# dropbox/lepton

Hardware: AMD Instinct MI355X
Metric: encode+decode MB/s (JPEG bytes/sec), bit-exact round trip (higher is better)
Workload: dtype int16/u8 (integer coder, no floating point)

## Files before the change

### lepton_amd/csrc/lep_enc5.h

```cpp
#pragma once
#include "lep_v3.h"
#ifdef LEP5_DEBUG
#include <cstdio>
#endif

namespace lep5 {
using namespace lep3;

constexpr int kRows = 64, kClasses = 10;
constexpr int kPRows = 63 + 14;
constexpr int kStreams = 2 * kRows * kClasses;
WDEV int stream_id(int ci, int row, int k) { return (ci * kRows + row) * kClasses + k; }
constexpr int kCoefSlice = 12 * 11 + 10 + 1;
constexpr int kSignSlice = 48, kNzSlice = 6 * 32, kEdgeNzSlice = 8 * 12, kDcSlice = 17 * 11 + 10 + 1;
constexpr uint32_t kThreshWords = 2u * 256 * 8 * 128;

WDEV uint32_t coef_entry(uint32_t vlow, int nres, int len, int bsr, int k, int u) {
    return vlow | ((uint32_t)nres << 10) | ((uint32_t)len << 14) | ((uint32_t)bsr << 18) | ((uint32_t)k << 23) | ((uint32_t)u << 27);
}
WDEV int coef_units(int len, int nres) { return ((len < 11 ? len + 1 : 11) + nres + 3) >> 2; }
WDEV uint32_t thresh_entry(uint32_t tbits, int n, int pcls, int lt, int u) {
    return tbits | ((uint32_t)n << 10) | ((uint32_t)pcls << 14) | ((uint32_t)lt << 23) | ((uint32_t)u << 27);
}
constexpr int kKeyRec = 4, kNzRec = 8, kEnRec = 8, kDcRec = 24;
// ... 413 lines not shown
                    if (overflow) status[sd.slot] = 100;
                } else { ws->low = bc.low; ws->stage = bc.stage; ws->q24 = bc.q24; ws->count = bc.count; ws->nst = bc.nst; ws->pos = bc.pos; }
            }
        }
    }
}


constexpr uint32_t kWarm5 = 16384;
struct WChunk5 { uint32_t q_guess, q_end, shifts, q_start, t_start, keep, keep_bits, carry, pos_end, pad[7]; };
static_assert(sizeof(WChunk5) == 64, "one record per (segment, chunk)");
WDEV uint32_t chunk_first_bin(uint32_t nbins, int k, int K) { return (uint32_t)(((uint64_t)nbins * (uint32_t)k) / (uint32_t)K); }
WDEV int range_step(uint32_t& q24, uint32_t bit, uint32_t prob) {
#if LEP_ON_GPU
    const uint32_t s = __umulhi(q24, prob);
#else
    const uint32_t s = (uint32_t)(((uint64_t)q24 * prob) >> 32);
#endif
    const uint32_t q = q24 >> 24;
    const uint32_t n = bit ? q - s : s + 1;
    const int f = __builtin_clz(n);
    q24 = (n << f) - (1u << 24);
    return f - 24;
}
template <class F, class G>
WDEV void for_bins(const uint16_t* list, uint32_t b0, uint32_t b1, F&& f, G&& g) {
    uint32_t i = b0;
    for (; i < b1 && (i & 31u); ++i) { const uint32_t e = list[i]; f((e >> 8) & 1u, e & 255u); g(); }
    if (i + 32 <= b1) {
        const uint32_t* b = reinterpret_cast<const uint32_t*>(list);
        U4 n0 = ld4(b + (i >> 1)), n1 = ld4(b + (i >> 1) + 4), n2 = ld4(b + (i >> 1) + 8), n3 = ld4(b + (i >> 1) + 12);
#define LEP5_BINS8(v)                                                                                      \
    f((v.x >> 8) & 1u, v.x & 255u); f((v.x >> 24) & 1u, (v.x >> 16) & 255u);                               \
    f((v.y >> 8) & 1u, v.y & 255u); f((v.y >> 24) & 1u, (v.y >> 16) & 255u); g();                          \
    f((v.z >> 8) & 1u, v.z & 255u); f((v.z >> 24) & 1u, (v.z >> 16) & 255u);                               \
    f((v.w >> 8) & 1u, v.w & 255u); f((v.w >> 24) & 1u, (v.w >> 16) & 255u); g();
        for (; i + 32 <= b1; i += 32) {
            const U4 g0 = n0, g1 = n1, g2 = n2, g3 = n3;
            const uint32_t* nx = b + (i >> 1) + 16;
            n0 = ld4(nx); n1 = ld4(nx + 4); n2 = ld4(nx + 8); n3 = ld4(nx + 12);
            LEP5_BINS8(g0) LEP5_BINS8(g1) LEP5_BINS8(g2) LEP5_BINS8(g3)
        }
#undef LEP5_BINS8
    }
    for (; i < b1; ++i) { const uint32_t e = list[i]; f((e >> 8) & 1u, e & 255u); g(); }
}
WDEV void range_run(const uint16_t* list, uint32_t b0, uint32_t b1, bool first, bool last, uint32_t& q24, uint32_t& shifts) {
    uint32_t t = 0, q = q24;
    if (first) t += (uint32_t)range_step(q, 0, 128);
    for_bins(list, b0, b1, [&](uint32_t bit, uint32_t prob) { t += (uint32_t)range_step(q, bit, prob); }, []() {});
    if (last) for (int i = 0; i < 32; ++i) t += (uint32_t)range_step(q, 0, 128);
    shifts = t; q24 = q;
}
WDEV void wchunk_range_lane(const SegPlan5& P, const uint16_t* bins, WChunk5* rec, int k, int K, uint32_t warm = kWarm5) {
    if (P.status) return;
    const uint16_t* list = bins + P.bins_off;
    const uint32_t b0 = chunk_first_bin(P.nbins, k, K), b1 = chunk_first_bin(P.nbins, k + 1, K);
    uint32_t q24 = 254u << 24, sh = 0;
    if (k > 0) {
        const bool from_start = b0 <= warm;
        range_run(list, from_start ? 0u : b0 - warm, b0, from_start, false, q24, sh);
    }
    rec->q_guess = q24;
    range_run(list, b0, b1, k == 0, k + 1 == K, q24, sh);
    rec->q_end = q24; rec->shifts = sh;
}
WDEV uint32_t bytes_at(uint32_t T) { return T >= 24 ? ((T - 24) >> 3) + 1 : 0u; }
WDEV int count_at(uint32_t T) { return (int)T - 24 - 8 * (int)bytes_at(T); }
WDEV void wchunk_link_lane(const SegPlan5& P, const uint16_t* bins, WChunk5* recs, int K) {
    if (P.status) return;
    const uint16_t* list = bins + P.bins_off;
    uint32_t T = 0, q = 254u << 24;
    for (int k = 0; k < K; ++k) {
        WChunk5& r = recs[k];
        if (k > 0 && r.q_guess != q) {
            uint32_t q24 = q, sh = 0;
            range_run(list, chunk_first_bin(P.nbins, k, K), chunk_first_bin(P.nbins, k + 1, K), false, k + 1 == K, q24, sh);
            r.q_end = q24; r.shifts = sh;
        }
        r.q_start = q; r.t_start = T;
        q = r.q_end; T += r.shifts;
    }
}
WDEV void wchunk_code_lane(const SegPlan5& P, const uint16_t* bins, const SegDev& sd, uint8_t* streams, WChunk5* rec, int k, int K) {
    if (P.status) return;
    const uint16_t* list = bins + P.bins_off;
    const uint32_t b0 = chunk_first_bin(P.nbins, k, K), b1 = chunk_first_bin(P.nbins, k + 1, K);
    BoolEnc5 bc;
    bc.init(streams + sd.stream_off, sd.stream_cap);
    bc.q24 = rec->q_start;
    bc.pos = bytes_at(rec->t_start); bc.count = count_at(rec->t_start); bc.floor_ = bc.pos;
    if (k == 0) { bc.bin(0, 128); bc.flush(); }
    for_bins(list, b0, b1, [&](uint32_t bit, uint32_t prob) { bc.bin(bit, prob); }, [&]() { bc.flush(); });
    bc.flush();
    if (k + 1 == K) for (int i = 0; i < 32; ++i) { bc.bin(0, 128); if ((i & 3) == 3) bc.flush(); }
    bc.flush();
    for (; bc.nst; --bc.nst) { if (bc.pos < bc.cap) bc.out[bc.pos] = (uint8_t)(bc.stage >> (8 * (bc.nst - 1))); ++bc.pos; }
    rec->keep = (uint32_t)bc.low; rec->keep_bits = (uint32_t)(32 + bc.count); rec->carry = bc.carry_out; rec->pos_end = bc.pos;
}
WDEV void add_back(uint8_t* out, uint32_t cap, uint32_t x, uint32_t v) {
    while (v && x > 0) {
        --x;
        if (x < cap) { const uint32_t t = out[x] + v; out[x] = (uint8_t)t; v = t >> 8; }
        else v = 0;
    }
}
WDEV void wchunk_stitch_lane(const SegPlan5& P, const SegDev& sd, uint8_t* streams, uint32_t* stream_len, int32_t* status, const WChunk5* recs, int K) {
    if (P.status) { status[sd.slot] = P.status; return; }
    uint8_t* out = streams + sd.stream_off;
    const uint32_t cap = sd.stream_cap;
    for (int k = 0; k + 1 < K; ++k) {
        const WChunk5& r = recs[k];
        const uint32_t X = r.keep_bits ? r.keep << (32 - r.keep_bits) : 0u;
        uint32_t carry = 0;
        for (int j = 3; j >= 0; --j) {
            const uint32_t x = r.pos_end + (uint32_t)j, add = (X >> (24 - 8 * j)) & 255u;
            if (x < cap) { const uint32_t t = out[x] + add + carry; out[x] = (uint8_t)t; carry = t >> 8; }
            else carry = 0;
        }
        add_back(out, cap, r.pos_end, carry);
        add_back(out, cap, recs[k + 1].t_start >= 24 ? bytes_at(recs[k + 1].t_start) : 0u, recs[k + 1].carry);
    }
    uint32_t pos = recs[K - 1].pos_end;
    const bool overflow = pos >= cap;
    if (!overflow && pos && (out[pos - 1] & 0xe0u) == 0xc0u) { out[pos] = 0; ++pos; }
    stream_len[sd.slot] = pos;
    if (overflow) status[sd.slot] = 100;
}

enum { kCount = 0, kEmit = 1, kGather = 2 };

#ifndef LEP_ENC5_GATHER_ROW_FLUSH
#define LEP_ENC5_GATHER_ROW_FLUSH 1
#endif
#if LEP_ENC5_GATHER_ROW_FLUSH
struct BinAcc {
    uint32_t lw;
    uint32_t fu;
    uint32_t blo, bhi;
};
#else
typedef uint32_t BinAcc;
#endif

struct Walk5Shared {
    uint32_t cur[32 * 65];
    uint16_t TB[8 * 65];
    uint16_t q[64];
    uint8_t thr[64];
    uint16_t errx[2 * 64];
    uint32_t tcur[2 * 8];
// ... 939 lines not shown
```

### lepton_amd/csrc/lep_gpu.hip

```cpp
#include <hip/hip_runtime.h>

#include <algorithm>
#include <cstdio>
#include <cstdlib>
#include <cstring>
#include <mutex>
#include <string>
#include <vector>

#include "../../include/lepton_mi355x.h"
#include "lep_buffers.h"

#define LEP_DEV __device__ __forceinline__
#include "lep_core.h"
#include "lep_enc3.h"
#include "lep_dec4.h"
#include "lep_enc5.h"
#include "lep_huff.h"
#include "lep_huffdec.h"
#include "lep_huffdec_simt.h"
#include "lep_huff_simt.h"
#include "lep_huffprog.h"
#include "lep_huffprog_simt.h"
#include "lep_huffprogdec.h"
// ... 131 lines not shown
    __shared__ lep4::Dec4Shared sh;
    const int s = blockIdx.x, lane = threadIdx.x;
    const SegDev seg = segs[s];
    lep4::Dec4Resume* rec = recs + seg.slot;
    const int state = rec->state;
    if (state != lep4::kRowsFresh && state != lep4::kRowsRunning) return;
    const ImageDev* img = images + seg.image;
    uint32_t* model = models + (size_t)s * kModelStride;
    NSum* ns = ns_area + ns_offsets[s];
    if (state == lep4::kRowsFresh) {
        reset_segment_state<lep3::kModelWords>(model, ns, img->ns_total, lane);
        __syncthreads();
    }
    lep4::Dec4WaveT<SCMASK> w;
#ifdef LEP_PROF
    w.prof_begin(&g_prof4[s & 8191][0]);
#endif
    w.run_rows(img, seg, model, ns, &sh, streams + seg.stream_off, stream_len[seg.slot], rec, lds_save + (size_t)seg.slot * kRowsLdsWords, band_mcu_rows);
}


template <int MODE, int NW>
__global__ __launch_bounds__(64 * NW) void lep_enc5_walk_kernel(const ImageDev* __restrict__ images, const SegDev* __restrict__ segs, NSum* ns_all,
                                                         const uint64_t* __restrict__ ns_off, lep5::SegPlan5* plans, uint8_t* arena, uint16_t* bins,
                                                         uint32_t* counts, int part, int nparts) {
    lep5::Walk5Shared* sh = reinterpret_cast<lep5::Walk5Shared*>(lep5::lep5_lds);
    const int s = blockIdx.x;
    const SegDev seg = segs[s];
    lep5::SegPlan5* P = plans + s;
    if (MODE == lep5::kGather && P->status) return;
    lep5::Walk5<MODE, NW> w;
    const int rc = w.run(images + seg.image, seg, ns_all + ns_off[s], sh, P, arena, bins, (int)(threadIdx.x >> 6), part, nparts);
    if (threadIdx.x >= 64) return;
    if (MODE == lep5::kCount) lep5::export_counts(w, sh, counts + (size_t)s * lep5::kCountWords);
    if (threadIdx.x == 0) {
        if (MODE == lep5::kEmit) P->status = rc;
        if (MODE == lep5::kGather && part + 1 == nparts) P->nbins = w.nbins;
    }
}
template <int PHASE>
__global__ __launch_bounds__(64) void lep_enc5_wchunk_kernel(const lep5::SegPlan5* __restrict__ plans, const uint16_t* __restrict__ bins, const SegDev* __restrict__ segs,
                                                         int nseg, int K, lep5::WChunk5* recs, uint8_t* streams, uint32_t* stream_len, int32_t* status, uint32_t* nbins_out) {
    const int id = (int)(blockIdx.x * 64 + threadIdx.x);
    if (PHASE == 0 || PHASE == 2) {
        const int seg = id / K, k = id - seg * K;
        if (seg >= nseg) return;
        if (PHASE == 2) __builtin_amdgcn_s_setprio(3);
        if (PHASE == 0) lep5::wchunk_range_lane(plans[seg], bins, recs + (size_t)seg * K + k, k, K);
        else lep5::wchunk_code_lane(plans[seg], bins, segs[seg], streams, recs + (size_t)seg * K + k, k, K);
    } else {
        if (id >= nseg) return;
        if (PHASE == 1) { status[segs[id].slot] = 0; nbins_out[segs[id].slot] = plans[id].nbins; lep5::wchunk_link_lane(plans[id], bins, recs + (size_t)id * K, K); }
        else lep5::wchunk_stitch_lane(plans[id], segs[id], streams, stream_len, status, recs + (size_t)id * K, K);
    }
}
__global__ void lep_enc5_plan_kernel(const uint32_t* __restrict__ counts, lep5::SegPlan5* plans, int nseg) {
    const int s = (int)(blockIdx.x * blockDim.x + threadIdx.x);
    if (s < nseg) lep5::plan_segment(counts + (size_t)s * lep5::kCountWords, plans + s);
}
__global__ __launch_bounds__(64) void lep_enc5_offsets_kernel(lep5::SegPlan5* plans, int nseg, uint64_t* totals) {
    uint64_t a = 0, b = 0;
    for (int s0 = 0; s0 < nseg; s0 += 64) {
        const int s = s0 + (int)threadIdx.x;
        const uint32_t ab = s < nseg ? plans[s].arena_bytes : 0u, bc = s < nseg ? plans[s].bins_cap : 0u;
        int oa, ob;
        const int va = (int)(ab >> 8), vb = (int)(bc >> 7);
        const int ta = lepwave::wave_excl_scan(&va, &oa), tb = lepwave::wave_excl_scan(&vb, &ob);
        if (s < nseg) { plans[s].arena_off = a + ((uint64_t)(uint32_t)oa << 8); plans[s].bins_off = b + ((uint64_t)(uint32_t)ob << 7); }
        a += (uint64_t)(uint32_t)ta << 8; b += (uint64_t)(uint32_t)tb << 7;
    }
    if (threadIdx.x == 0) { totals[0] = a; totals[1] = b; }
}
__global__ void lep_enc5_fill_kernel(uint4* p, size_t n16, uint32_t v) {
    const uint4 x = make_uint4(v, v, v, v);
    for (size_t i = blockIdx.x * (size_t)blockDim.x + threadIdx.x; i < n16; i += (size_t)gridDim.x * blockDim.x) p[i] = x;
}
__global__ __launch_bounds__(64) void lep_enc5_bucket_kernel(const lep5::SegPlan5* __restrict__ plans, uint8_t* arena) {
    __shared__ lep5::BucketShared sh;
    lep5::bucket_wave(plans + blockIdx.x, arena, &sh);
}
struct Fold5CoefShared { uint16_t slice[lep5::kCoefSlice * 64]; };
__global__ __launch_bounds__(64) void lep_enc5_fold_coef_kernel(const lep5::SegPlan5* __restrict__ plans, uint8_t* arena, int nseg, int groups) {
    __shared__ Fold5CoefShared shc;
    const int grp = (int)blockIdx.x % groups, job = (int)blockIdx.x / groups;
    const int ci = job / 630, row = (job % 630) / 10, k = job % 10;
    const int sid = lep5::stream_id(ci, row, k), seg = grp * 64 + (int)threadIdx.x;
    const bool work = seg < nseg && !plans[seg].status && plans[seg].cnt[sid] != 0;
    if (!__ballot(work)) return;
    lep5::fold_coef_wave(plans, arena, grp * 64, nseg, sid, reinterpret_cast<lep5::FoldShared*>(&shc));
}
struct Fold5SmallShared { uint16_t slice[lep5::kEdgeNzSlice * 64]; };
__global__ __launch_bounds__(64) void lep_enc5_fold_small_kernel(const lep5::SegPlan5* __restrict__ plans, uint8_t* arena, uint32_t* thresh_models, int nseg, int groups, int job0) {
    __shared__ Fold5SmallShared shs;
    lep5::FoldShared* sh = reinterpret_cast<lep5::FoldShared*>(&shs);
    const int grp = (int)blockIdx.x % groups;
    int job = (int)blockIdx.x / groups + job0;
    const int seg0 = grp * 64;
    if (job < 2) { lep5::fold_sign_wave(plans, arena, seg0, nseg, job, sh); return; }
    job -= 2;
    if (job < 12) { const int ci = job / 6, lt = 2 + job % 6; lep5::fold_thresh_wave(plans, arena, thresh_models, seg0, nseg, lep5::stream_id(ci, 63, lt), ci, sh); return; }
    job -= 12;
    lep5::fold_edgenz_wave(plans, arena, seg0, nseg, job / 16, (job / 8) & 1, job & 7, sh);
}
constexpr int kFold5SmallJobs = 2 + 12 + 32;
__global__ __launch_bounds__(64) void lep_enc5_fold_big_kernel(const lep5::SegPlan5* __restrict__ plans, uint8_t* arena, int nseg, int groups, int job0) {
    __shared__ lep5::FoldShared sh;
// ... 191 lines not shown
    __shared__ lephuff::SimtShared sh;
    extern __shared__ __attribute__((aligned(16))) unsigned char simt_columns[];
    const lephuff::SimtWave w = waves[blockIdx.x];
    lephuff::simt_guess_or_settle(images + w.image, &sh, si + w.image, in + si[w.image].first, out + si[w.image].first, w.first_sub, settle, slots,
                                  reinterpret_cast<lephuff::SimtColumns*>(simt_columns));
}
__global__ __launch_bounds__(64) void lep_huffman_simt_place_kernel(const lephuff::HuffDecImage* __restrict__ images, lephuff::SimtImage* si, const lephuff::SimtSub* sub,
                                                                    lephuff::SimtPlace* place, int passes, lephuff::HuffDecRow* rows, const lephuff::SimtSlots* slots) {
    const int i = (int)blockIdx.x;
    lephuff::simt_place(images + i, si + i, sub + si[i].first, place + si[i].first, passes, rows, slots);
}
__global__ __launch_bounds__(64) void lep_huffman_simt_write_kernel(const lephuff::HuffDecImage* __restrict__ images, lephuff::SimtImage* si, const lephuff::SimtWave* waves,
                                                                    const lephuff::SimtSub* sub, const lephuff::SimtPlace* place, lephuff::HuffDecRow* rows) {
    __shared__ lephuff::SimtShared sh;
    __shared__ lephuff::SimtTile tile;
    const lephuff::SimtWave w = waves[blockIdx.x];
    lephuff::simt_write(images + w.image, &sh, &tile, si + w.image, sub + si[w.image].first, place + si[w.image].first, rows, w.first_sub);
}
__global__ void lep_huffman_simt_finish_kernel(const lephuff::HuffDecImage* __restrict__ images, int nimg, lephuff::HuffDecRow* rows, const lephuff::SimtImage* si) {
    const int i = (int)(blockIdx.x * blockDim.x + threadIdx.x);
    if (i < nimg) lephuff::simt_finish(images + i, si + i, rows);
}

}

struct lep_gpu {
    int device = 0;
    hipStream_t stream = nullptr;
    hipEvent_t ev0 = nullptr, ev1 = nullptr;
    bool timed = false;
    bool released = false;
    int enc5_min = 8;
    hipStream_t stream2 = nullptr, stream3 = nullptr;
    hipEvent_t ev_fork = nullptr, ev_join = nullptr, ev_join3 = nullptr;
    int huffprog_pipeline = 1;
    int huffprog_split = 0;
    int huffprogdec_rst = 1;
    uint32_t huffprogdec_rst_floor = lephuff::kRstPieceFloor;
    int huffprogdec_win = 1;
    int huffprog_simt = 1;
    int huffprog_simt_rst = 1;
    uint32_t huffprog_forms[4] = {0, 0, 0, 0};
    int cut_progressive = 0;
    int stream_pack = 1;
    int huffenc_simt = 1;
    int simt_sub_bits = 0;
    int huffprog_pipeline_max = 16384;
    int enc5_waves = 2;
    int enc5_parts = 8;
    hipEvent_t ev_part[8] = {nullptr, nullptr, nullptr, nullptr, nullptr, nullptr, nullptr, nullptr};
    long enc5_wlanes = 131072;
    int enc5_wmaxseg = 4096;
    int enc5_wchunks = 64;
    int enc5_gather_wgs = 0;
    int enc5_fold_apart = 0;
    size_t enc5_scratch_max = ~(size_t)0;
    hipEvent_t ev_stage[8] = {nullptr, nullptr, nullptr, nullptr, nullptr, nullptr, nullptr, nullptr};
    int nstage = 0;
    int enc_waves = 0;
    int enc_pair_max = 1280;
    int dec_company = 0;
    int dec_waves = 0;
    std::string err;
    const char* last_kernel = "";
    char simt_name[112] = "";
    struct Vmm {
        bool on = false;
        size_t chunk = (size_t)512 << 20;
        hipMemAllocationProp prop;
        hipMemAccessDesc access;
        std::vector<hipMemGenericAllocationHandle_t> pool;
        size_t mapped_total = 0, creates = 0, releases = 0;
    } vmm;
    enum Ws {
        W_ENC5_ENTRIES,
        W_ENC5_BINLIST,
        W_MODELS, W_MODELS_1,
        W_NS, W_NS_1,
        W_TRIMMED,
        W_META = W_TRIMMED, W_META_1,
        W_ROWS, W_ROWS_1,
        W_ENC5_PLANS,
        W_ENC5_WCHUNKS,
        W_BLOCKS, W_STREAMS, W_LENS,
        W_HUFF, W_HUFF_1,
        W_HUFFENC, W_HUFFENC_1,
        W_HUFFPROG, W_HUFFPROG_1,
        W_HUFFPROGSIMT, W_HUFFPROGSIMT_1,
        W_HUFFSEQ, W_HUFFSEQ_1,
        W_HUFFPROGDEC,
        W_HUFFPROGRST,
        W_HUFFDEC,
        W_HUFFPAR,
        W_PACK, W_PACK_1,
        W_COUNT
    };
    lepbuf::DevBuf<> ws[W_COUNT];
    int cur = 0;
    struct RowsSession {
        bool open = false;
        int nseg = 0, waves = 4;
        hipStream_t st = nullptr;
        const ImageDev* d_img = nullptr; const SegDev* d_seg = nullptr; const uint64_t* d_nsoff = nullptr;
        uint32_t* d_models = nullptr; NSum* d_ns = nullptr;
        const uint8_t* d_streams = nullptr; const uint32_t* d_stream_len = nullptr;
        std::vector<lep4::Dec4Resume> h_recs;
// ... 106 lines not shown
        if (hipMemMap(b.va + b.mapped, V.chunk, 0, h, 0) != hipSuccess) { (void)hipGetLastError(); (void)hipMemRelease(h); g->err = "hipMemMap failed"; return LEP_GPU_ERROR; }
        b.chunks.push_back(h); b.mapped += V.chunk; V.mapped_total += V.chunk;
    }
    if (b.mapped > old) HIPCHK(g, hipMemSetAccess(b.va + old, b.mapped - old, &V.access, 1));
    w.set(b.va, b.mapped);
    return 0;
}
static int ensure(lep_gpu* g, Workspace& w, size_t need, bool may_release = true) {
    if (w.cap >= need) return 0;
    if (g->vmm.on && (need >= ((size_t)32 << 20) || w.v.va)) {
        if (!w.v.va) HIPCHK(g, w.release());
        return vmm_ensure(g, w, need, may_release);
    }
    hipError_t e = w.ensure(need, need / 8);
    if (e != hipSuccess && may_release) {
        (void)hipGetLastError();
        release_idle_caches(g);
        e = w.ensure(need);
    }
    if (e != hipSuccess) { g->err = std::string("hipMalloc: ") + hipGetErrorString(e); return LEP_GPU_ERROR; }
    return 0;
}

#include "lep_derive.h"


constexpr int kEnc5NoMemory = -1000;
static int launch_enc5(lep_gpu* g, const ImageDev* d_img, const SegDev* d_seg, const uint64_t* d_nsoff, int nseg, uint8_t* d_streams,
                       uint32_t* d_stream_len, int32_t* d_status, hipStream_t st) {
    Workspace &models = g->ws[lep_gpu::W_MODELS + g->cur], &ns = g->ws[lep_gpu::W_NS + g->cur];
    Workspace &ws_plans = g->ws[lep_gpu::W_ENC5_PLANS], &ws_entries = g->ws[lep_gpu::W_ENC5_ENTRIES], &ws_binlist = g->ws[lep_gpu::W_ENC5_BINLIST], &wchunks = g->ws[lep_gpu::W_ENC5_WCHUNKS];
    if (!g->stream2) {
        HIPCHK(g, hipEventCreateWithFlags(&g->ev_enc5_done, hipEventDisableTiming));
        for (auto& e : g->ev_part) HIPCHK(g, hipEventCreateWithFlags(&e, hipEventDisableTiming));
        HIPCHK(g, hipStreamCreateWithFlags(&g->stream2, hipStreamNonBlocking));
        HIPCHK(g, hipStreamCreateWithFlags(&g->stream3, hipStreamNonBlocking));
        HIPCHK(g, hipEventCreateWithFlags(&g->ev_fork, hipEventDisableTiming));
        HIPCHK(g, hipEventCreateWithFlags(&g->ev_join, hipEventDisableTiming));
        HIPCHK(g, hipEventCreateWithFlags(&g->ev_join3, hipEventDisableTiming));
        for (auto& e : g->ev_stage) HIPCHK(g, hipEventCreate(&e));
    }
    lepbuf::Layout L;
    L.add<lep5::SegPlan5>((size_t)nseg);
    const size_t o_counts = L.add<uint32_t>((size_t)nseg * lep5::kCountWords), o_tot = L.add<uint64_t>(2);
    HIPCHK(g, hipStreamWaitEvent(st, g->ev_enc5_done, 0));
    if (int rc = ensure(g, ws_plans, L.padded())) return rc;
    lep5::SegPlan5* plans = ws_plans.at<lep5::SegPlan5>(0);
    uint32_t* counts = ws_plans.at<uint32_t>(o_counts);
    uint64_t* d_tot = ws_plans.at<uint64_t>(o_tot);
    const int groups = (nseg + 63) / 64;
    g->nstage = 0;
    HIPCHK(g, hipEventRecord(g->ev_stage[0], st));
    const bool two = g->enc5_waves == 2;
    const int nparts = std::min(std::max(g->enc5_parts, 1), (int)lep5::kMaxParts);
    auto walk = [&](int mode, uint8_t* entries, uint16_t* binlist, int part = 0) {
        size_t lds = lep5::walk_lds_bytes(mode);
        if (mode == lep5::kGather && g->enc5_gather_wgs > 0) lds = std::max(lds, (size_t)(160 * 1024 / g->enc5_gather_wgs) & ~(size_t)255);
#define LEP_WALK(MODE, NW) hipLaunchKernelGGL((lep_enc5_walk_kernel<MODE, NW>), dim3(nseg), dim3(64 * NW), lds, st, d_img, d_seg, (NSum*)ns.p, d_nsoff, plans, entries, binlist, counts, part, nparts)
        if (mode == lep5::kCount) { if (two) LEP_WALK(lep5::kCount, 2); else LEP_WALK(lep5::kCount, 1); }
        else if (mode == lep5::kEmit) { if (two) LEP_WALK(lep5::kEmit, 2); else LEP_WALK(lep5::kEmit, 1); }
        else { if (two) LEP_WALK(lep5::kGather, 2); else LEP_WALK(lep5::kGather, 1); }
#undef LEP_WALK
    };
    walk(lep5::kCount, nullptr, nullptr);
    hipLaunchKernelGGL(lep_enc5_plan_kernel, dim3(groups), dim3(64), 0, st, (const uint32_t*)counts, plans, nseg);
    hipLaunchKernelGGL(lep_enc5_offsets_kernel, dim3(1), dim3(64), 0, st, plans, nseg, d_tot);
    hipLaunchKernelGGL(lep_enc5_fill_kernel, dim3(4096), dim3(256), 0, st, (uint4*)models.p, (size_t)nseg * lep5::kThreshWords / 4, kBranchInit);
    uint64_t tot[2] = {0, 0};
    HIPCHK(g, hipMemcpyAsync(tot, d_tot, sizeof tot, hipMemcpyDeviceToHost, st));
    HIPCHK(g, hipStreamSynchronize(st));
    if ((size_t)tot[0] + (size_t)tot[1] * 2 > g->enc5_scratch_max || ensure(g, ws_entries, (size_t)tot[0] + 256, false) || ensure(g, ws_binlist, (size_t)tot[1] * 2 + 256, false)) {
        (void)hipGetLastError();
        g->err.clear();
        static bool told = false;
        if (!told) { told = true; fprintf(stderr, "lepton-mi355x: no room for the split-phase encoder's scratch (%.1f GB for %d segments): single-kernel encoder\n", ((double)tot[0] + 2.0 * (double)tot[1]) / 1e9, nseg); }
        return kEnc5NoMemory;
    }
    {
        HIPCHK(g, hipEventRecord(g->ev_stage[1], st));
        walk(lep5::kEmit, (uint8_t*)ws_entries.p, nullptr);
        HIPCHK(g, hipEventRecord(g->ev_stage[2], st));
        hipLaunchKernelGGL(lep_enc5_bucket_kernel, dim3(nseg), dim3(64), 0, st, (const lep5::SegPlan5*)plans, (uint8_t*)ws_entries.p);
        HIPCHK(g, hipEventRecord(g->ev_fork, st));
        HIPCHK(g, hipStreamWaitEvent(g->stream2, g->ev_fork, 0));
        HIPCHK(g, hipStreamWaitEvent(g->stream3, g->ev_fork, 0));
        if (g->enc5_fold_apart) {
            const int small0[4] = {0, 2, 14, 46}, big0[3] = {0, 12, 32};
            for (int i = 0; i < 3; ++i)
                hipLaunchKernelGGL(lep_enc5_fold_small_kernel, dim3((unsigned)groups * (small0[i + 1] - small0[i])), dim3(64), 0, st, (const lep5::SegPlan5*)plans, (uint8_t*)ws_entries.p,
                                   (uint32_t*)models.p, nseg, groups, small0[i]);
            for (int i = 0; i < 2; ++i)
                hipLaunchKernelGGL(lep_enc5_fold_big_kernel, dim3((unsigned)groups * (big0[i + 1] - big0[i])), dim3(64), 0, st, (const lep5::SegPlan5*)plans, (uint8_t*)ws_entries.p, nseg, groups, big0[i]);
        } else {
        hipLaunchKernelGGL(lep_enc5_fold_small_kernel, dim3((unsigned)groups * kFold5SmallJobs), dim3(64), 0, g->stream2, (const lep5::SegPlan5*)plans, (uint8_t*)ws_entries.p,
                           (uint32_t*)models.p, nseg, groups, 0);
        hipLaunchKernelGGL(lep_enc5_fold_big_kernel, dim3((unsigned)groups * kFold5BigJobs), dim3(64), 0, g->stream3, (const lep5::SegPlan5*)plans, (uint8_t*)ws_entries.p, nseg, groups, 0);
        }
        hipLaunchKernelGGL(lep_enc5_fold_coef_kernel, dim3((unsigned)groups * 1260u), dim3(64), 0, st, (const lep5::SegPlan5*)plans, (uint8_t*)ws_entries.p, nseg, groups);
        HIPCHK(g, hipEventRecord(g->ev_join, g->stream2));
        HIPCHK(g, hipEventRecord(g->ev_join3, g->stream3));
        HIPCHK(g, hipStreamWaitEvent(st, g->ev_join, 0));
        HIPCHK(g, hipStreamWaitEvent(st, g->ev_join3, 0));
        HIPCHK(g, hipEventRecord(g->ev_stage[3], st));
        int K = 0;
        if (g->enc5_wchunks >= 2 && nseg <= g->enc5_wmaxseg) { K = 1; while (K * 2 <= g->enc5_wchunks && (long)nseg * K * 2 <= g->enc5_wlanes) K *= 2; }
        if (K >= 2 && ensure(g, wchunks, (size_t)nseg * K * sizeof(lep5::WChunk5) + 256, false)) { (void)hipGetLastError(); g->err.clear(); K = 0; }
        if (K >= 2) {
            for (int part = 0; part < nparts; ++part) walk(lep5::kGather, (uint8_t*)ws_entries.p, (uint16_t*)ws_binlist.p, part);
            HIPCHK(g, hipEventRecord(g->ev_stage[4], st));
            lep5::WChunk5* recs = (lep5::WChunk5*)wchunks.p;
            const int lane_groups = (int)(((long)nseg * K + 63) / 64);
#define LEP_WCHUNK(PHASE, GRID) hipLaunchKernelGGL((lep_enc5_wchunk_kernel<PHASE>), dim3(GRID), dim3(64), 0, st, (const lep5::SegPlan5*)plans, (const uint16_t*)ws_binlist.p, d_seg, nseg, K, recs, d_streams, d_stream_len, d_status, g->d_bins)
            LEP_WCHUNK(0, lane_groups); LEP_WCHUNK(1, groups); LEP_WCHUNK(2, lane_groups); LEP_WCHUNK(3, groups);
#undef LEP_WCHUNK
            HIPCHK(g, hipEventRecord(g->ev_stage[5], st));
            g->nstage = 5;
        } else {
        for (int part = 0; part < nparts; ++part) {
            walk(lep5::kGather, (uint8_t*)ws_entries.p, (uint16_t*)ws_binlist.p, part);
            HIPCHK(g, hipEventRecord(g->ev_part[part], st));
            HIPCHK(g, hipStreamWaitEvent(g->stream2, g->ev_part[part], 0));
            hipLaunchKernelGGL(lep_enc5_write_kernel, dim3(groups), dim3(64), 0, g->stream2, (const lep5::SegPlan5*)plans, (const uint16_t*)ws_binlist.p, d_seg, nseg, d_streams,
                               d_stream_len, d_status, g->d_bins, (uint8_t*)ws_entries.p, part, nparts);
        }
        HIPCHK(g, hipEventRecord(g->ev_stage[4], st));
        HIPCHK(g, hipEventRecord(g->ev_join, g->stream2));
        HIPCHK(g, hipStreamWaitEvent(st, g->ev_join, 0));
        HIPCHK(g, hipEventRecord(g->ev_stage[5], st));
        g->nstage = 5;
        }
    }
    HIPCHK(g, hipEventRecord(g->ev_enc5_done, st));
    HIPCHK(g, hipGetLastError());
    g->last_kernel = "lep_enc5 (count | emit | fold | gather | write)";
    return 0;
}

static int upload(lep_gpu* g, void* dst, const void* src, size_t n, hipStream_t st) {
    if (!n) return 0;
    lep_gpu::Staging& sl = g->staging[g->staging_next];
    g->staging_next = (g->staging_next + 1) % 16;
    if (sl.used) { HIPCHK(g, hipEventSynchronize(sl.ev)); sl.used = false; }
    if (!sl.ev) HIPCHK(g, hipEventCreateWithFlags(&sl.ev, hipEventDisableTiming));
    if (sl.cap < n) {
        if (sl.host) g->staging_retired.push_back(sl.host);
        sl.host = nullptr; sl.cap = 0;
        const size_t want = std::max<size_t>(n + n / 4 + 4096, (size_t)8 << 20);
        HIPCHK(g, hipHostMalloc(&sl.host, want, hipHostMallocDefault));
        sl.cap = want;
    }
    memcpy(sl.host, src, n);
    HIPCHK(g, hipMemcpyAsync(dst, sl.host, n, hipMemcpyHostToDevice, st));
    HIPCHK(g, hipEventRecord(sl.ev, st));
    sl.used = true;
    return 0;
}

static int refuse_if_session(lep_gpu* g, const char* what) {
    if (!g->rows[g->cur].open) return 0;
    g->err = std::string(what) + ": arena set " + std::to_string(g->cur) + " belongs to a decode session until lep_gpu_decode_rows_end";
    return LEP_ASSERTION_FAILURE;
}

struct LaunchFront { const ImageDev* d_img; const SegDev* d_seg; const uint64_t* d_nsoff; uint32_t* d_models; NSum* d_ns; };
static int launch_front(lep_gpu* g, bool dec, const lep_image_desc* images, int nimg, const lep_segment* segs, int nseg,
                        const uint64_t* stream_offsets, hipStream_t st, LaunchFront* out) {
    std::vector<ImageDev> himg(nimg);
    for (int i = 0; i < nimg; ++i) {
        int rc = derive_image(images[i], &himg[i], !dec);
        if (rc) return rc;
    }
    std::vector<SegDev> hseg(nseg);
    std::vector<uint64_t> hns(nseg);
    uint64_t ns_total = 0;
    for (int s = 0; s < nseg; ++s)
        if (segs[s].image < 0 || segs[s].image >= nimg) return LEP_ASSERTION_FAILURE;
    const bool permute = nseg > 8;
    std::vector<int> order(nseg);
    if (permute) {
        std::vector<int> q[8];
        int rank = 0;
        for (int s = 0; s < nseg; ++s) {
            rank = (s > 0 && segs[s].image == segs[s - 1].image) ? rank + 1 : 0;
            q[(rank + segs[s].image) & 7].push_back(s);
        }
        size_t at[8] = {0, 0, 0, 0, 0, 0, 0, 0};
        for (int i = 0; i < nseg;)
// ... 89 lines not shown
        }
        if (done) {}
        else if (waves == 2) {
            g->last_kernel = "lep_encode_v3x2_kernel";
            hipLaunchKernelGGL(lep_encode_v3x2_kernel, dim3(nseg), dim3(128), 0, st, F.d_img, F.d_seg, (uint32_t*)models.p, (NSum*)ns.p, F.d_nsoff,
                               d_streams, d_stream_len, d_status, g->d_bins);
        }
        else if (waves >= 8) { g->last_kernel = "lep_encode_v3_kernel<8>"; LEP_LAUNCH_ENC3(8); }
        else { g->last_kernel = "lep_encode_v3_kernel<4>"; LEP_LAUNCH_ENC3(4); }
#undef LEP_LAUNCH_ENC3
    }
    HIPCHK(g, hipGetLastError());
    HIPCHK(g, hipEventRecord(g->ev1, st));
    g->timed = true;
    return 0;
}

__attribute__((constructor)) static void lep_runtime_defaults() { setenv("GPU_MAX_HW_QUEUES", "8", 0); }

extern "C" {

static std::mutex g_live_mu;
static std::vector<lep_gpu*> g_live;
static bool g_exit_hook = false;
static void release_device_side(lep_gpu* g);
static void release_all_at_exit() {
    std::lock_guard<std::mutex> lk(g_live_mu);
    for (lep_gpu* g : g_live) release_device_side(g);
    g_live.clear();
}

int lep_gpu_create(int device, lep_gpu** out) {
    lep_gpu* g = new lep_gpu;
    g->device = device;
    if (const char* e = getenv("LEP_DEC_WAVES")) g->dec_waves = atoi(e) == 4 ? 4 : (atoi(e) == 8 ? 8 : 0);
    if (const char* e = getenv("LEP_ENC_WAVES")) g->enc_waves = atoi(e) == 4 ? 4 : (atoi(e) == 8 ? 8 : (atoi(e) == 2 ? 2 : 0));
    if (const char* e = getenv("LEP_ENC_PAIR_MAX")) g->enc_pair_max = atoi(e);
    if (const char* e = getenv("LEP_ENC5_MIN")) g->enc5_min = atoi(e);
    if (const char* e = getenv("LEP_HUFFPROG_PIPELINE")) g->huffprog_pipeline = atoi(e);
    if (const char* e = getenv("LEP_HUFFPROG_PIPELINE_MAX")) g->huffprog_pipeline_max = atoi(e);
    if (const char* e = getenv("LEP_HUFFDEC_SIMT_BITS")) g->simt_sub_bits = std::max(0, atoi(e));
    if (const char* e = getenv("LEP_HUFFENC_SIMT")) g->huffenc_simt = atoi(e) != 0;
    if (const char* e = getenv("LEP_STREAM_PACK")) g->stream_pack = atoi(e) != 0;
    if (const char* e = getenv("LEP_CUT_PROGRESSIVE")) g->cut_progressive = atoi(e) != 0;
    if (const char* e = getenv("LEP_HUFFPROG_SIMT")) g->huffprog_simt = atoi(e) != 0;
    if (const char* e = getenv("LEP_HUFFPROG_SIMT_RST")) g->huffprog_simt_rst = atoi(e) != 0;
    if (const char* e = getenv("LEP_HUFFPROGDEC_WIN")) g->huffprogdec_win = atoi(e) != 0;
    if (const char* e = getenv("LEP_HUFFPROGDEC_RST")) g->huffprogdec_rst = atoi(e) != 0;
    if (const char* e = getenv("LEP_HUFFPROGDEC_RST_FLOOR")) g->huffprogdec_rst_floor = (uint32_t)std::max(1, atoi(e));
    if (const char* e = getenv("LEP_HUFFPROG_SPLIT")) g->huffprog_split = atoi(e) != 0;
    if (const char* e = getenv("LEP_ENC5_WAVES")) g->enc5_waves = atoi(e) == 1 ? 1 : 2;
    if (const char* e = getenv("LEP_ENC5_FOLD_APART")) g->enc5_fold_apart = atoi(e);
    if (const char* e = getenv("LEP_ENC5_GATHER_WGS")) g->enc5_gather_wgs = atoi(e);
    if (const char* e = getenv("LEP_ENC5_PARTS")) g->enc5_parts = atoi(e);
    if (const char* e = getenv("LEP_ENC5_WCHUNKS")) g->enc5_wchunks = atoi(e);
    if (const char* e = getenv("LEP_ENC5_WLANES")) g->enc5_wlanes = atol(e);
    if (const char* e = getenv("LEP_ENC5_WMAXSEG")) g->enc5_wmaxseg = atoi(e);
    if (const char* e = getenv("LEP_ENC5_SCRATCH_MAX")) g->enc5_scratch_max = (size_t)strtoull(e, nullptr, 10);
    int n = 0;
    if (hipGetDeviceCount(&n) != hipSuccess || n <= device) { delete g; return LEP_GPU_ERROR; }
    if (hipSetDevice(device) != hipSuccess || hipStreamCreate(&g->stream) != hipSuccess ||
        hipEventCreate(&g->ev0) != hipSuccess || hipEventCreate(&g->ev1) != hipSuccess) { delete g; return LEP_GPU_ERROR; }
    vmm_init(g);
    {
        std::lock_guard<std::mutex> lk(g_live_mu);
        g_live.push_back(g);
        if (!g_exit_hook) { g_exit_hook = true; atexit(release_all_at_exit); }
    }
    *out = g;
    return 0;
}

static void release_device_side(lep_gpu* g) {
    if (g->released) return;
    g->released = true;
    (void)hipSetDevice(g->device);
    (void)hipStreamSynchronize(g->stream);
    if (g->ev_enc5_done) (void)hipEventDestroy(g->ev_enc5_done);
    for (auto& e : g->ev_part) if (e) (void)hipEventDestroy(e);
    for (auto& e : g->ev_stage) if (e) (void)hipEventDestroy(e);
    if (g->ev_fork) (void)hipEventDestroy(g->ev_fork);
    if (g->ev_join) (void)hipEventDestroy(g->ev_join);
    if (g->ev_join3) (void)hipEventDestroy(g->ev_join3);
    if (g->stream2) (void)hipStreamDestroy(g->stream2);
    if (g->stream3) (void)hipStreamDestroy(g->stream3);
    for (Workspace& w : g->ws) dev_release(g, w);
    vmm_destroy(g);
    if (g->ev0) (void)hipEventDestroy(g->ev0);
    if (g->ev1) (void)hipEventDestroy(g->ev1);
    if (g->stream) (void)hipStreamDestroy(g->stream);
    for (auto& h : g->h_huffprog) (void)h.release();
    for (lep_gpu::Staging& sl : g->staging) { if (sl.host) (void)hipHostFree(sl.host); if (sl.ev) (void)hipEventDestroy(sl.ev); sl = lep_gpu::Staging(); }
    for (void* p : g->staging_retired) (void)hipHostFree(p);
    g->staging_retired.clear();
}

void lep_gpu_destroy(lep_gpu* g) {
    if (!g) return;
    {
        std::lock_guard<std::mutex> lk(g_live_mu);
        for (size_t i = 0; i < g_live.size(); ++i) if (g_live[i] == g) { g_live.erase(g_live.begin() + i); break; }
        release_device_side(g);
    }
    delete g;
}

const char* lep_gpu_last_error(lep_gpu* g) { return g ? g->err.c_str() : "no gpu object"; }

int lep_gpu_encode_device(lep_gpu* g, const lep_image_desc* images, int nimg, const lep_segment* segs, int nseg,
                          uint8_t* d_streams, const uint64_t* stream_offsets, uint32_t* d_stream_len, int32_t* d_status,
// ... 680 lines not shown
```

Before: 1701.

## Run per-part range-coder chunk kernels on a second stream beside gather

Adds a part-aware chunked range-coder schedule that launches range, link and code kernels per gather part on a side stream, so arithmetic coding overlaps with later gather walks. Chunk boundaries come from per-part checkpoints. The default scheduling also changes: the chunked path no longer switches off above the max segment count, and gather is forced to a single part when chunking is active unless parts were given. The aim is to hide gather latency behind coding, at the cost of more launches and event syncs.

```diff
diff --git a/lepton_amd/csrc/lep_enc5.h b/lepton_amd/csrc/lep_enc5.h
--- a/lepton_amd/csrc/lep_enc5.h
+++ b/lepton_amd/csrc/lep_enc5.h
@@ -489,51 +489,67 @@
     if (last) for (int i = 0; i < 32; ++i) t += (uint32_t)range_step(q, 0, 128);
     shifts = t; q24 = q;
 }
-WDEV void wchunk_range_lane(const SegPlan5& P, const uint16_t* bins, WChunk5* rec, int k, int K, uint32_t warm = kWarm5) {
+struct ChunkCut5 { uint32_t b0, b1; bool first, last; };
+WDEV ChunkCut5 chunk_cut(uint32_t nbins, int k, int K) { return ChunkCut5{chunk_first_bin(nbins, k, K), chunk_first_bin(nbins, k + 1, K), k == 0, k + 1 == K}; }
+WDEV ChunkCut5 part_chunk_cut(const SegPlan5& P, const Ckpt5* ck, int p, int s, int nparts, int c) {
+    const uint32_t B0 = p > 0 ? ck[p].nbins : 0u, B1 = p + 1 < nparts ? ck[p + 1].nbins : P.nbins, d = B1 - B0;
+    return ChunkCut5{B0 + chunk_first_bin(d, s, c), B0 + chunk_first_bin(d, s + 1, c), p == 0 && s == 0, p + 1 == nparts && s + 1 == c};
+}
+WDEV void wchunk_range_cut(const SegPlan5& P, const uint16_t* bins, WChunk5* rec, const ChunkCut5& c, uint32_t warm = kWarm5) {
     if (P.status) return;
     const uint16_t* list = bins + P.bins_off;
-    const uint32_t b0 = chunk_first_bin(P.nbins, k, K), b1 = chunk_first_bin(P.nbins, k + 1, K);
     uint32_t q24 = 254u << 24, sh = 0;
-    if (k > 0) {
-        const bool from_start = b0 <= warm;
-        range_run(list, from_start ? 0u : b0 - warm, b0, from_start, false, q24, sh);
+    if (!c.first) {
+        const bool from_start = c.b0 <= warm;
+        range_run(list, from_start ? 0u : c.b0 - warm, c.b0, from_start, false, q24, sh);
     }
     rec->q_guess = q24;
-    range_run(list, b0, b1, k == 0, k + 1 == K, q24, sh);
+    range_run(list, c.b0, c.b1, c.first, c.last, q24, sh);
     rec->q_end = q24; rec->shifts = sh;
+}
+WDEV void wchunk_range_lane(const SegPlan5& P, const uint16_t* bins, WChunk5* rec, int k, int K, uint32_t warm = kWarm5) {
+    wchunk_range_cut(P, bins, rec, chunk_cut(P.nbins, k, K), warm);
 }
 WDEV uint32_t bytes_at(uint32_t T) { return T >= 24 ? ((T - 24) >> 3) + 1 : 0u; }
 WDEV int count_at(uint32_t T) { return (int)T - 24 - 8 * (int)bytes_at(T); }
-WDEV void wchunk_link_lane(const SegPlan5& P, const uint16_t* bins, WChunk5* recs, int K) {
+template <class CUT>
+WDEV void wchunk_link_cuts(const SegPlan5& P, const uint16_t* bins, WChunk5* recs, int j0, int j1, CUT&& cut) {
     if (P.status) return;
     const uint16_t* list = bins + P.bins_off;
     uint32_t T = 0, q = 254u << 24;
-    for (int k = 0; k < K; ++k) {
-        WChunk5& r = recs[k];
-        if (k > 0 && r.q_guess != q) {
+    if (j0 > 0) { q = recs[j0 - 1].q_end; T = recs[j0 - 1].t_start + recs[j0 - 1].shifts; }
+    for (int j = j0; j < j1; ++j) {
+        WChunk5& r = recs[j];
+        if (j > 0 && r.q_guess != q) {
+            const ChunkCut5 c = cut(j);
             uint32_t q24 = q, sh = 0;
-            range_run(list, chunk_first_bin(P.nbins, k, K), chunk_first_bin(P.nbins, k + 1, K), false, k + 1 == K, q24, sh);
+            range_run(list, c.b0, c.b1, false, c.last, q24, sh);
             r.q_end = q24; r.shifts = sh;
         }
         r.q_start = q; r.t_start = T;
         q = r.q_end; T += r.shifts;
     }
 }
-WDEV void wchunk_code_lane(const SegPlan5& P, const uint16_t* bins, const SegDev& sd, uint8_t* streams, WChunk5* rec, int k, int K) {
+WDEV void wchunk_link_lane(const SegPlan5& P, const uint16_t* bins, WChunk5* recs, int K) {
+    wchunk_link_cuts(P, bins, recs, 0, K, [&](int k) { return chunk_cut(P.nbins, k, K); });
+}
+WDEV void wchunk_code_cut(const SegPlan5& P, const uint16_t* bins, const SegDev& sd, uint8_t* streams, WChunk5* rec, const ChunkCut5& c) {
     if (P.status) return;
     const uint16_t* list = bins + P.bins_off;
-    const uint32_t b0 = chunk_first_bin(P.nbins, k, K), b1 = chunk_first_bin(P.nbins, k + 1, K);
     BoolEnc5 bc;
     bc.init(streams + sd.stream_off, sd.stream_cap);
     bc.q24 = rec->q_start;
     bc.pos = bytes_at(rec->t_start); bc.count = count_at(rec->t_start); bc.floor_ = bc.pos;
-    if (k == 0) { bc.bin(0, 128); bc.flush(); }
-    for_bins(list, b0, b1, [&](uint32_t bit, uint32_t prob) { bc.bin(bit, prob); }, [&]() { bc.flush(); });
+    if (c.first) { bc.bin(0, 128); bc.flush(); }
+    for_bins(list, c.b0, c.b1, [&](uint32_t bit, uint32_t prob) { bc.bin(bit, prob); }, [&]() { bc.flush(); });
     bc.flush();
-    if (k + 1 == K) for (int i = 0; i < 32; ++i) { bc.bin(0, 128); if ((i & 3) == 3) bc.flush(); }
+    if (c.last) for (int i = 0; i < 32; ++i) { bc.bin(0, 128); if ((i & 3) == 3) bc.flush(); }
     bc.flush();
     for (; bc.nst; --bc.nst) { if (bc.pos < bc.cap) bc.out[bc.pos] = (uint8_t)(bc.stage >> (8 * (bc.nst - 1))); ++bc.pos; }
     rec->keep = (uint32_t)bc.low; rec->keep_bits = (uint32_t)(32 + bc.count); rec->carry = bc.carry_out; rec->pos_end = bc.pos;
+}
+WDEV void wchunk_code_lane(const SegPlan5& P, const uint16_t* bins, const SegDev& sd, uint8_t* streams, WChunk5* rec, int k, int K) {
+    wchunk_code_cut(P, bins, sd, streams, rec, chunk_cut(P.nbins, k, K));
 }
 WDEV void add_back(uint8_t* out, uint32_t cap, uint32_t x, uint32_t v) {
     while (v && x > 0) {
diff --git a/lepton_amd/csrc/lep_gpu.hip b/lepton_amd/csrc/lep_gpu.hip
--- a/lepton_amd/csrc/lep_gpu.hip
+++ b/lepton_amd/csrc/lep_gpu.hip
@@ -207,6 +207,25 @@
         if (id >= nseg) return;
         if (PHASE == 1) { status[segs[id].slot] = 0; nbins_out[segs[id].slot] = plans[id].nbins; lep5::wchunk_link_lane(plans[id], bins, recs + (size_t)id * K, K); }
         else lep5::wchunk_stitch_lane(plans[id], segs[id], streams, stream_len, status, recs + (size_t)id * K, K);
+    }
+}
+template <int PHASE>
+__global__ __launch_bounds__(64) void lep_enc5_wchunk_part_kernel(const lep5::SegPlan5* __restrict__ plans, const uint16_t* __restrict__ bins, const SegDev* __restrict__ segs,
+                                                              int nseg, int nparts, int c, int part, lep5::WChunk5* recs, uint8_t* streams, const uint8_t* __restrict__ arena,
+                                                              int32_t* status, uint32_t* nbins_out) {
+    __builtin_amdgcn_s_setprio(3);
+    const int id = (int)(blockIdx.x * 64 + threadIdx.x);
+    const int seg = PHASE == 1 ? id : id / c, s = PHASE == 1 ? 0 : id - seg * c;
+    if (seg >= nseg) return;
+    const lep5::SegPlan5& P = plans[seg];
+    const lep5::Ckpt5* ck = reinterpret_cast<const lep5::Ckpt5*>(arena + P.arena_off + P.ckpt_base);
+    lep5::WChunk5* r = recs + (size_t)seg * (size_t)(nparts * c);
+    if (PHASE == 0) lep5::wchunk_range_cut(P, bins, r + part * c + s, lep5::part_chunk_cut(P, ck, part, s, nparts, c));
+    else if (PHASE == 2) lep5::wchunk_code_cut(P, bins, segs[seg], streams, r + part * c + s, lep5::part_chunk_cut(P, ck, part, s, nparts, c));
+    else {
+        if (part == 0) status[segs[seg].slot] = 0;
+        if (part + 1 == nparts) nbins_out[segs[seg].slot] = P.nbins;
+        lep5::wchunk_link_cuts(P, bins, r, part * c, (part + 1) * c, [&](int j) { return lep5::part_chunk_cut(P, ck, j / c, j % c, nparts, c); });
     }
 }
 __global__ void lep_enc5_plan_kernel(const uint32_t* __restrict__ counts, lep5::SegPlan5* plans, int nseg) {
@@ -504,6 +523,9 @@
     long enc5_wlanes = 131072;
     int enc5_wmaxseg = 4096;
     int enc5_wchunks = 64;
+    bool enc5_parts_given = false;
+    int enc5_wsched = 1;
+    int enc5_wpartchunks = 4;
     int enc5_gather_wgs = 0;
     int enc5_fold_apart = 0;
     size_t enc5_scratch_max = ~(size_t)0;
@@ -716,8 +738,11 @@
     g->nstage = 0;
     HIPCHK(g, hipEventRecord(g->ev_stage[0], st));
     const bool two = g->enc5_waves == 2;
-    const int nparts = std::min(std::max(g->enc5_parts, 1), (int)lep5::kMaxParts);
-    auto walk = [&](int mode, uint8_t* entries, uint16_t* binlist, int part = 0) {
+    const int wsched = nseg <= g->enc5_wmaxseg ? 1 : g->enc5_wsched;
+    int K = 0;
+    if (g->enc5_wchunks >= 2 && wsched == 1) { K = 1; while (K * 2 <= g->enc5_wchunks && (long)nseg * K * 2 <= g->enc5_wlanes) K *= 2; }
+    int nparts = std::min(std::max(g->enc5_parts, 1), (int)lep5::kMaxParts);
+    auto walk =[&](int mode, uint8_t* entries, uint16_t* binlist, int part = 0) {
         size_t lds = lep5::walk_lds_bytes(mode);
         if (mode == lep5::kGather && g->enc5_gather_wgs > 0) lds = std::max(lds, (size_t)(160 * 1024 / g->enc5_gather_wgs) & ~(size_t)255);
 #define LEP_WALK(MODE, NW) hipLaunchKernelGGL((lep_enc5_walk_kernel<MODE, NW>), dim3(nseg), dim3(64 * NW), lds, st, d_img, d_seg, (NSum*)ns.p, d_nsoff, plans, entries, binlist, counts, part, nparts)
@@ -740,6 +765,12 @@
         if (!told) { told = true; fprintf(stderr, "lepton-mi355x: no room for the split-phase encoder's scratch (%.1f GB for %d segments): single-kernel encoder\n", ((double)tot[0] + 2.0 * (double)tot[1]) / 1e9, nseg); }
         return kEnc5NoMemory;
     }
+    if (K >= 2 && ensure(g, wchunks, (size_t)nseg * K * sizeof(lep5::WChunk5) + 256, false)) { (void)hipGetLastError(); g->err.clear(); K = 0; }
+    if (K >= 2 && !g->enc5_parts_given) nparts = 1;
+    const int c = wsched == 2 ? g->enc5_wpartchunks : 0;
+    const bool beside = c >= 1 && !ensure(g, wchunks, (size_t)nseg * nparts * c * sizeof(lep5::WChunk5) + 256, false);
+    if (c >= 1 && !beside) { (void)hipGetLastError(); g->err.clear(); }
+    const bool wrote_beside = beside;
     {
         HIPCHK(g, hipEventRecord(g->ev_stage[1], st));
         walk(lep5::kEmit, (uint8_t*)ws_entries.p, nullptr);
@@ -766,10 +797,26 @@
         HIPCHK(g, hipStreamWaitEvent(st, g->ev_join, 0));
         HIPCHK(g, hipStreamWaitEvent(st, g->ev_join3, 0));
         HIPCHK(g, hipEventRecord(g->ev_stage[3], st));
-        int K = 0;
-        if (g->enc5_wchunks >= 2 && nseg <= g->enc5_wmaxseg) { K = 1; while (K * 2 <= g->enc5_wchunks && (long)nseg * K * 2 <= g->enc5_wlanes) K *= 2; }
-        if (K >= 2 && ensure(g, wchunks, (size_t)nseg * K * sizeof(lep5::WChunk5) + 256, false)) { (void)hipGetLastError(); g->err.clear(); K = 0; }
-        if (K >= 2) {
+        if (beside) {
+            lep5::WChunk5* recs = (lep5::WChunk5*)wchunks.p;
+            const int lane_groups = (int)(((long)nseg * c + 63) / 64);
+#define LEP_WPART(PHASE, GRID) hipLaunchKernelGGL((lep_enc5_wchunk_part_kernel<PHASE>), dim3(GRID), dim3(64), 0, g->stream2, (const lep5::SegPlan5*)plans, (const uint16_t*)ws_binlist.p, d_seg, nseg, \
+                                                  nparts, c, part, recs, d_streams, (const uint8_t*)ws_entries.p, d_status, g->d_bins)
+            for (int part = 0; part < nparts; ++part) {
+                walk(lep5::kGather, (uint8_t*)ws_entries.p, (uint16_t*)ws_binlist.p, part);
+                HIPCHK(g, hipEventRecord(g->ev_part[part], st));
+                HIPCHK(g, hipStreamWaitEvent(g->stream2, g->ev_part[part], 0));
+                LEP_WPART(0, lane_groups); LEP_WPART(1, groups); LEP_WPART(2, lane_groups);
+            }
+#undef LEP_WPART
+            HIPCHK(g, hipEventRecord(g->ev_stage[4], st));
+            hipLaunchKernelGGL((lep_enc5_wchunk_kernel<3>), dim3(groups), dim3(64), 0, g->stream2, (const lep5::SegPlan5*)plans, (const uint16_t*)ws_binlist.p, d_seg, nseg, nparts * c, recs,
+                               d_streams, d_stream_len, d_status, g->d_bins);
+            HIPCHK(g, hipEventRecord(g->ev_join, g->stream2));
+            HIPCHK(g, hipStreamWaitEvent(st, g->ev_join, 0));
+            HIPCHK(g, hipEventRecord(g->ev_stage[5], st));
+            g->nstage = 5;
+        } else if (K >= 2) {
             for (int part = 0; part < nparts; ++part) walk(lep5::kGather, (uint8_t*)ws_entries.p, (uint16_t*)ws_binlist.p, part);
             HIPCHK(g, hipEventRecord(g->ev_stage[4], st));
             lep5::WChunk5* recs = (lep5::WChunk5*)wchunks.p;
@@ -796,7 +843,7 @@
     }
     HIPCHK(g, hipEventRecord(g->ev_enc5_done, st));
     HIPCHK(g, hipGetLastError());
-    g->last_kernel = "lep_enc5 (count | emit | fold | gather | write)";
+    g->last_kernel = wrote_beside ? "lep_enc5 (count | emit | fold | gather | write: part chunks beside gather)" : "lep_enc5 (count | emit | fold | gather | write)";
     return 0;
 }
 
@@ -992,10 +1039,12 @@
     if (const char* e = getenv("LEP_ENC5_WAVES")) g->enc5_waves = atoi(e) == 1 ? 1 : 2;
     if (const char* e = getenv("LEP_ENC5_FOLD_APART")) g->enc5_fold_apart = atoi(e);
     if (const char* e = getenv("LEP_ENC5_GATHER_WGS")) g->enc5_gather_wgs = atoi(e);
-    if (const char* e = getenv("LEP_ENC5_PARTS")) g->enc5_parts = atoi(e);
+    if (const char* e = getenv("LEP_ENC5_PARTS")) { g->enc5_parts = atoi(e); g->enc5_parts_given = true; }
     if (const char* e = getenv("LEP_ENC5_WCHUNKS")) g->enc5_wchunks = atoi(e);
     if (const char* e = getenv("LEP_ENC5_WLANES")) g->enc5_wlanes = atol(e);
     if (const char* e = getenv("LEP_ENC5_WMAXSEG")) g->enc5_wmaxseg = atoi(e);
+    if (const char* e = getenv("LEP_ENC5_WSCHED")) g->enc5_wsched = !strcmp(e, "lane") ? 0 : !strcmp(e, "after") ? 1 : !strcmp(e, "beside") ? 2 : std::min(std::max(atoi(e), 0), 2);
+    if (const char* e = getenv("LEP_ENC5_WPARTCHUNKS")) { const int c = atoi(e); g->enc5_wpartchunks = 1; while (g->enc5_wpartchunks * 2 <= std::min(c, 32)) g->enc5_wpartchunks *= 2; }
     if (const char* e = getenv("LEP_ENC5_SCRATCH_MAX")) g->enc5_scratch_max = (size_t)strtoull(e, nullptr, 10);
     int n = 0;
     if (hipGetDeviceCount(&n) != hipSuccess || n <= device) { delete g; return LEP_GPU_ERROR; }
```

Result: faster. 1742 (median of 6 runs) (+2.4%).
